# balazs-bamer/cdpr-simulation

Measured on AMD Instinct MI355X. Metric: CDPR sim-steps/sec (whole node), 65 536 parallel 8-cable robots, 1 ms dt, higher is better.
Workload: dtype f32

## Files before the change

### cdpr-simulation_amd/csrc/cdpr_onestep_kernel.hpp

```cpp
#pragma once
#include "cdpr_step_kernel.hpp"

namespace cdpr {

CDPR_DEV void row_to_lds(const float4* src, float4* dst_row) {
  __builtin_amdgcn_global_load_lds((const __attribute__((address_space(1))) void*)src, (__attribute__((address_space(3))) void*)dst_row, 16, 0, 0);
}


template <int NP, bool PR = false, bool FULL = false>
CDPR_DEV void pid_pairs(const StepArgs& a, int calls, bool is_vel, const v2f (&desired)[NP], const v2f (&actual)[NP], const v2f (&win)[NP][kWin],
                        v2f (&ierr)[NP], v2f (&f)[NP], v2f (&e_new)[NP], float& dbg_p, float& dbg_i, float& dbg_d, bool is_force = false) {
  const PidCoef c = pid_coef<PR>(a, is_vel);
  const bool run = (!PR || calls != 0) && !is_force;
  const bool full = FULL || calls >= c.nbuf;
  const float (&wt)[kWin + 2] = a.wrow;
  v2f error[NP], acc[NP];
#pragma unroll
  for (int k = 0; k < NP; ++k) {
    error[k] = desired[k] - actual[k];
    acc[k] = splat(wt[kWin]) * error[k];
  }
#pragma unroll
  for (int j = 0; j < kWin; ++j) {
#pragma unroll
    for (int k = 0; k < NP; ++k) acc[k] = fma2(wt[j], win[k][j], acc[k]);
  }
#pragma unroll
  for (int k = 0; k < NP; ++k) {
    const v2f p_term = splat(c.kp) * error[k];
    const v2f prev_ierr = ierr[k];
    v2f ie = fma2(a.dt, error[k], prev_ierr);
    const v2f i_term = splat(c.ki) * ie;
    const v2f i_cl = max2(min2(i_term, splat(c.imax)), splat(c.imin));
    const v2f ie_cl = i_cl * splat(c.inv_ki);
    ie.x = (i_cl.x != i_term.x) ? ie_cl.x : ie.x;
    ie.y = (i_cl.y != i_term.y) ? ie_cl.y : ie.y;
    const v2f derived = full ? acc[k] * splat(a.inv_dt) : splat(0.f);
    const v2f d_term = splat(c.kd) * derived;
    const v2f cmd = fma2(c.kf, desired[k], p_term) + i_cl + d_term;
    v2f out = c.clamp ? max2(min2(cmd, splat(c.cmax)), splat(c.cmin)) : cmd;
    const v2f bumped = fma2(splat(a.dt) * error[k], splat(c.ki), out);
    ie.x = (out.x != cmd.x) ? prev_ierr.x : ie.x;
    ie.y = (out.y != cmd.y) ? prev_ierr.y : ie.y;
    out.x = (out.x != cmd.x) ? bumped.x : out.x;
    out.y = (out.y != cmd.y) ? bumped.y : out.y;
    ierr[k] = run ? ie : prev_ierr;
    f[k] = run ? out : (is_force ? desired[k] : splat(0.f));
    e_new[k] = error[k];
    if (k == 0) {
      dbg_p = p_term.x;
      dbg_i = i_term.x;
      dbg_d = d_term.x;
    }
  }
}

typedef float f32x4 __attribute__((ext_vector_type(4)));
CDPR_DEV f32x4 load_slot_untracked(const float4* base, size_t stride, int slot, uint32_t off) {
  const char* p = reinterpret_cast<const char*>(base + (size_t)slot * stride) + off;
  f32x4 v;
  asm volatile("global_load_dwordx4 %0, %1, off" : "=a"(v) : "v"(p) : "memory");
  return v;
}
constexpr int vmcnt_imm(int n) { return (n & 15) | ((n >> 4) << 14) | (7 << 4) | (15 << 8); }

template <int N, bool FK, bool TD, bool PERSIST = false>
__global__ __launch_bounds__(64, 1) void cdpr_onestep_kernel(const StepArgs a_in) {
  const StepArgs& a = a_in;
  constexpr int NP = cable_pairs(N);
  constexpr int P = plat_slots(FK);
  constexpr int G = joint_groups(N);
  constexpr int NH = (NP + 1) / 2;
  constexpr int kCtrl = 5 * NP + NH;
  constexpr bool kCmdLds = (N % 4) == 0;
  constexpr int kCmdRows = kCmdLds ? N / 4 : 0;
  __shared__ __attribute__((aligned(16))) float lds[NP * kGeomFloatsPerPair];
  __shared__ float4 stage[kCtrl + (kCmdRows ? kCmdRows : 1)][64];

  const uint32_t lane = threadIdx.x;
  const size_t st0 = a.stride;
  const uint32_t nblocks = (a.batch + 63u) / 64u;
  uint32_t blk = blockIdx.x;
  uint32_t r = blk * 64u + lane;
  uint32_t rr = (r < a.batch) ? r : (a.batch - 1u);
  bool live = r < a.batch;
  uint32_t off = rr * 16u, woff = r * 16u;

  CDPR_STAMP(0);
  const float gval = (lane < NP * kGeomFloatsPerPair) ? a.geom[lane] : 0.f;
  float4 p0 = load_slot(a.state, st0, 0, off), p1 = load_slot(a.state, st0, 1, off), p2 = load_slot(a.state, st0, 2, off),
         p3 = load_slot(a.state, st0, 3, off);
  float4 p4 = make_float4(0.f, 0.f, 0.f, 1.f);
  if (FK) p4 = load_slot(a.state, st0, 4, off);
  if (lane < NP * kGeomFloatsPerPair) lds[lane] = gval;
  const bool force_mode = (a.flags & kFlagForceMode) != 0u;
  const bool first_world = (a.flags & kFlagFirstWorldStep) != 0u;
  const bool run_pid = !first_world && !force_mode && a.pid_calls != 0;
  bool staged = false;

  for (;;) {
  size_t st = st0;
  uint32_t goff = 0;
  if (PERSIST) asm volatile("" : "+s"(st), "+v"(goff));
  const float* const geo = lds + goff;
  const StepArgs a = block_args<PERSIST>(a_in);
  v2f desired[NP];
#pragma unroll
  for (int k = 0; k < NP; ++k) desired[k] = splat(0.f);
  const float* cp = a.cmd + (size_t)rr * N;
  if (!kCmdLds || force_mode) {
#pragma unroll
    for (int i = 0; i < N; ++i) {
      if (i & 1)
        desired[i / 2].y = cp[i];
      else
        desired[i / 2].x = cp[i];
    }
  }
  __builtin_amdgcn_fence(__ATOMIC_RELEASE, "wavefront");
  __builtin_amdgcn_wave_barrier();
  __builtin_amdgcn_fence(__ATOMIC_ACQUIRE, "wavefront");

  Platform s;
  unpack_platform(p0, p1, p2, p3.x, s);
  float fkx = p3.y, fky = p3.z, fkz = p3.w, fkqx = p4.x, fkqy = p4.y, fkqz = p4.z, fkqw = p4.w;

  {
    float keep = (s.px + s.qy) + (s.vy + s.wz) + fkqw;
#pragma unroll
    for (int k = 0; k < NP; ++k) keep += desired[k].x + desired[k].y;
    asm volatile("" ::"v"(keep));
    if (run_pid && !staged) {
#pragma unroll
      for (int j = 0; j < kCtrl; ++j)
        row_to_lds(reinterpret_cast<const float4*>(reinterpret_cast<const char*>(a.state + (size_t)(P + j) * st) + off), &stage[j][0]);
      if (kCmdLds) {
#pragma unroll
        for (int g = 0; g < kCmdRows; ++g) row_to_lds(reinterpret_cast<const float4*>(cp) + g, &stage[kCtrl + g][0]);
      }
    }
  }

  const uint32_t nblk = blk + gridDim.x;
  const bool more = PERSIST && nblk < nblocks;
  uint32_t nr = 0, nrr = 0;
  f32x4 n0 = {0.f, 0.f, 0.f, 0.f}, n1 = n0, n2 = n0, n3 = n0, n4 = {0.f, 0.f, 0.f, 1.f};
  if (PERSIST && more) {
    nr = nblk * 64u + lane;
    nrr = (nr < a.batch) ? nr : (a.batch - 1u);
    const uint32_t noff = nrr * 16u;
    n0 = load_slot_untracked(a.state, st, 0, noff), n1 = load_slot_untracked(a.state, st, 1, noff);
    n2 = load_slot_untracked(a.state, st, 2, noff), n3 = load_slot_untracked(a.state, st, 3, noff);
    if (FK) n4 = load_slot_untracked(a.state, st, 4, noff);
  }

  CDPR_STAMP(1);
  v2f len[NP], q[NP], qd[NP], jac[NP][6];
  {
    v2f l0[NP];
    ik_pairs<N, true>(geo, s.px, s.py, s.pz, s.qx, s.qy, s.qz, s.qw, len, jac, l0);
#pragma unroll
    for (int k = 0; k < NP; ++k) {
      q[k] = l0[k] - len[k];
      qd[k] = -fma2(s.wz, jac[k][5], fma2(s.wy, jac[k][4], fma2(s.wx, jac[k][3],
                    fma2(s.vz, jac[k][2], fma2(s.vy, jac[k][1], splat(s.vx) * jac[k][0])))));
    }
  }
  const bool publish = (a.publish_mask & 1ull) != 0ull;
  if (publish && live) {
    store_slot(a.obs, st, 0, woff, make_float4(s.px, s.py, s.pz, s.qx));
    store_slot(a.obs, st, 1, woff, make_float4(s.qy, s.qz, s.qw, s.vx));
    store_slot(a.obs, st, 2, woff, make_float4(s.vy, s.vz, s.wx, s.wy));
#pragma unroll
    for (int g = 0; g < G; ++g) {
      const int k0 = 2 * g, k1 = (2 * g + 1 < NP) ? 2 * g + 1 : 2 * g;
      const bool has = (2 * g + 1 < NP);
      store_slot(a.obs, st, 4 + g, woff, make_float4(q[k0].x, q[k0].y, has ? q[k1].x : 0.f, has ? q[k1].y : 0.f));
      store_slot(a.obs, st, 4 + G + g, woff, make_float4(qd[k0].x, qd[k0].y, has ? qd[k1].x : 0.f, has ? qd[k1].y : 0.f));
    }
  }

  CDPR_STAMP(2);
  float fk_res = 0.f;
  int fk_it = 0;
  v2f jest[NP][6];
  if (FK) {
    v2f elen[NP], unused[NP];
    bool active = true;
    for (int it = 0; it < a.fk_iters; ++it) {
      ik_pairs<N, false>(geo, fkx, fky, fkz, fkqx, fkqy, fkqz, fkqw, elen, jest, unused);
      v2f res[NP];
      v2f rm = splat(0.f);
#pragma unroll
      for (int k = 0; k < NP; ++k) {
        res[k] = len[k] - elen[k];
        rm = max2(rm, abs2(res[k]));
      }
      active = active && !(fmaxf(rm.x, rm.y) < a.fk_tol);
      float g[6];
      jt_times<NP>(jest, res, g);
      normal_solve<NP>(jest, a.fk_lambda, g);
      if (active) {
        fkx += g[0];
        fky += g[1];
        fkz += g[2];
        quat_apply_rotvec(fkqx, fkqy, fkqz, fkqw, g[3], g[4], g[5]);
        ++fk_it;
      }
    }
    ik_pairs<N, false>(geo, fkx, fky, fkz, fkqx, fkqy, fkqz, fkqw, elen, jest, unused);
    v2f rm = splat(0.f);
#pragma unroll
    for (int k = 0; k < NP; ++k) rm = max2(rm, abs2(len[k] - elen[k]));
    fk_res = fmaxf(rm.x, rm.y);
  }

  CDPR_STAMP(3);
  v2f f[NP], e_new[NP], ierr[NP];
#pragma unroll
  for (int k = 0; k < NP; ++k) {
    f[k] = splat(0.f);
    e_new[k] = splat(0.f);
    ierr[k] = splat(0.f);
  }
  float dbg_p = 0.f, dbg_i = 0.f, dbg_d = 0.f;
  bool dbg_wrote = false;
  if (run_pid) {
    __builtin_amdgcn_s_waitcnt(0x0F70);
    __builtin_amdgcn_fence(__ATOMIC_ACQUIRE, "wavefront");
    CDPR_STAMP(4);
    if (kCmdLds) {
#pragma unroll
      for (int g = 0; g < kCmdRows; ++g) {
        const float4 v = stage[kCtrl + g][lane];
        desired[2 * g] = (v2f){v.x, v.y};
        desired[2 * g + 1] = (v2f){v.z, v.w};
      }
    }
    v2f win[NP][kWin];
#pragma unroll
    for (int k = 0; k < NP; ++k) {
#pragma unroll
      for (int m = 0; m < 5; ++m) {
        const float4 w = stage[5 * k + m][lane];
        win[k][2 * m] = (v2f){w.x, w.y};
        win[k][2 * m + 1] = (v2f){w.z, w.w};
      }
    }
#pragma unroll
    for (int g = 0; g < NH; ++g) {
      const float4 h = stage[5 * NP + g][lane];
      ierr[2 * g] = (v2f){h.x, h.y};
      if (2 * g + 1 < NP) ierr[2 * g + 1] = (v2f){h.z, h.w};
    }
    const bool actual_is_vel = (a.flags & kFlagActualIsVelocity) != 0u;
    v2f actual[NP];
#pragma unroll
    for (int k = 0; k < NP; ++k) actual[k] = actual_is_vel ? qd[k] : q[k];
    const int ring_slot = a.ring_slot;
    pid_pairs<NP>(a, a.pid_calls, actual_is_vel, desired, actual, win, ierr, f, e_new, dbg_p, dbg_i, dbg_d);
    dbg_wrote = true;
    if (live) {
#pragma unroll
      for (int m = 0; m < 5; ++m) {
        if (m == (ring_slot >> 1)) {
#pragma unroll
          for (int k = 0; k < NP; ++k) CDPR_STORE_STATE(a.state, st, P + 5 * k + m, woff, ring_row(win[k], m, e_new[k], ring_slot));
        }
      }
#pragma unroll
      for (int g = 0; g < NH; ++g) {
        const int k1 = (2 * g + 1 < NP) ? 2 * g + 1 : 2 * g;
        CDPR_STORE_STATE(a.state, st, P + 5 * NP + g, woff, make_float4(ierr[2 * g].x, ierr[2 * g].y, ierr[k1].x, ierr[k1].y));
      }
    }
  }

  if (force_mode && !first_world) {
#pragma unroll
    for (int k = 0; k < NP; ++k) f[k] = desired[k];
  }

  if (PERSIST && more) {
    const uint32_t noff = nrr * 16u;
    if (run_pid) {
#pragma unroll
      for (int j = 0; j < kCtrl; ++j)
        row_to_lds(reinterpret_cast<const float4*>(reinterpret_cast<const char*>(a.state + (size_t)(P + j) * st) + noff), &stage[j][0]);
      if (kCmdLds) {
        const float* ncp = a.cmd + (size_t)nrr * N;
#pragma unroll
        for (int g = 0; g < kCmdRows; ++g) row_to_lds(reinterpret_cast<const float4*>(ncp) + g, &stage[kCtrl + g][0]);
      }
    }
  }

  CDPR_STAMP(5);
  v2f applied[NP];
  int td_flag = 0;
  if (TD) {
    v2f df[NP];
#pragma unroll
    for (int k = 0; k < NP; ++k) df[k] = f[k] - splat(a.td_mid);
    float g[6];
    if (FK) {
      jt_times<NP>(jest, df, g);
      normal_solve<NP, false>(jest, 0.f, g);
    } else {
      jt_times<NP>(jac, df, g);
      normal_solve<NP, false>(jac, 0.f, g);
    }
#pragma unroll
    for (int k = 0; k < NP; ++k) {
      v2f t = splat(a.td_mid);
#pragma unroll
      for (int c = 0; c < 6; ++c) t = fma2(g[c], FK ? jest[k][c] : jac[k][c], t);
      const v2f tc = max2(min2(t, splat(a.td_max)), splat(a.td_min));
      td_flag |= (tc.x != t.x) ? 1 : 0;
      if (2 * k + 1 < N) td_flag |= (tc.y != t.y) ? 1 : 0;
      applied[k] = tc;
    }
  } else {
#pragma unroll
    for (int k = 0; k < NP; ++k) applied[k] = f[k];
  }
  setforce_limits<NP>(a, qd, applied);

  if (a.dbg && live) write_pid_topic(a.dbg + (size_t)r * 9, dbg_wrote, dbg_wrote, dbg_p, dbg_i, dbg_d, desired[0].x, applied[0].x);
  if (publish && live) {
    store_slot(a.obs, st, 3, woff, make_float4(s.wz, fk_res, (float)fk_it, pack_flags(td_flag, travel_mask<N>(a, q))));
#pragma unroll
    for (int g = 0; g < G; ++g) {
      const int k0 = 2 * g, k1 = (2 * g + 1 < NP) ? 2 * g + 1 : 2 * g;
      const bool has = (2 * g + 1 < NP);
      store_slot(a.obs, st, 4 + 2 * G + g, woff,
                make_float4(applied[k0].x, applied[k0].y, has ? applied[k1].x : 0.f, has ? applied[k1].y : 0.f));
    }
  }

  CDPR_STAMP(6);
  {
    v2f tens[NP];
#pragma unroll
    for (int k = 0; k < NP; ++k) {
      tens[k] = fma2(-a.damping, qd[k], applied[k]);
      if (a.unilateral) tens[k] = max2(tens[k], splat(0.f));
    }
    if (FK) {
      uint32_t again = 0;
      asm volatile("" : "+v"(again));
      v2f len2[NP], l02[NP];
      ik_pairs<N, false>(lds + again, s.px, s.py, s.pz, s.qx, s.qy, s.qz, s.qw, len2, jac, l02);
    }
    float w[6];
    jt_times<NP>(jac, tens, w);
    w[0] = a.fgx - w[0];
    w[1] = a.fgy - w[1];
    w[2] = a.fgz - w[2];
    w[3] = -w[3];
    w[4] = -w[4];
    w[5] = -w[5];
    integrate(a, s, w);
  }
  if (PERSIST && more) {
    constexpr int kDmaOps = kCtrl + kCmdRows;
    static_assert(kDmaOps < 64, "vmcnt is a 6-bit counter");
    if (run_pid)
      __builtin_amdgcn_s_waitcnt(vmcnt_imm(kDmaOps));
    else
      __builtin_amdgcn_s_waitcnt(vmcnt_imm(0));
    asm volatile("" : "+a"(n0), "+a"(n1), "+a"(n2), "+a"(n3), "+a"(n4));
  }
  if (live) {
    CDPR_STORE_STATE(a.state, st, 0, woff, make_float4(s.px, s.py, s.pz, s.qx));
    CDPR_STORE_STATE(a.state, st, 1, woff, make_float4(s.qy, s.qz, s.qw, s.vx));
    CDPR_STORE_STATE(a.state, st, 2, woff, make_float4(s.vy, s.vz, s.wx, s.wy));
    CDPR_STORE_STATE(a.state, st, 3, woff, make_float4(s.wz, fkx, fky, fkz));
    if (FK) CDPR_STORE_STATE(a.state, st, 4, woff, make_float4(fkqx, fkqy, fkqz, fkqw));
  }
  CDPR_STAMP(7);
  if (!(PERSIST && more)) break;
  blk = nblk;
  r = nr;
  rr = nrr;
  live = r < a.batch;
  off = rr * 16u, woff = r * 16u;
  p0 = make_float4(n0.x, n0.y, n0.z, n0.w), p1 = make_float4(n1.x, n1.y, n1.z, n1.w), p2 = make_float4(n2.x, n2.y, n2.z, n2.w);
  p3 = make_float4(n3.x, n3.y, n3.z, n3.w), p4 = make_float4(n4.x, n4.y, n4.z, n4.w);
  staged = run_pid;
  }
}

#ifndef CDPR_CTL_LOAD_DELAY
#define CDPR_CTL_LOAD_DELAY 8
#endif
#ifndef CDPR_SPLIT_PRIO
#define CDPR_SPLIT_PRIO 1
#endif
#ifndef CDPR_STEADY_SHARED_IK
#define CDPR_STEADY_SHARED_IK 1
#endif
#ifndef CDPR_STEADY_NEWTON_WRITTEN_OUT
#define CDPR_STEADY_NEWTON_WRITTEN_OUT 1
#endif
constexpr int kIkRows = 7;
#ifdef CDPR_STAMPS
#define CDPR_SPLIT_STAMP(i)                                                                                          \
  do {                                                                                                               \
    __builtin_amdgcn_sched_barrier(0);                                                                               \
    if (a.stamps && lane == 0) a.stamps[(size_t)blockIdx.x * 8 + (i)] = __builtin_amdgcn_s_memrealtime();           \
    __builtin_amdgcn_sched_barrier(0);                                                                               \
  } while (0)
#else
#define CDPR_SPLIT_STAMP(i) do { } while (0)
#endif
#if defined(CDPR_STAMPS) && defined(CDPR_STAMPS_ITER)
#define CDPR_CTL_STAMP(i) do { } while (0)
#else
#define CDPR_CTL_STAMP(i) CDPR_SPLIT_STAMP(i)
#endif

template <int N, int XS, int ES, bool RAISED = true, bool STEADY = false>
CDPR_DEV void split_estimator_wave(const StepArgs& a, float* geo, float gval, uint32_t lane, bool live, size_t st, uint32_t off, uint32_t woff,
                                   const float4& p0, const float4& p1, const float4& p3, const v2f* x_force, v2f* x_tension, float* x_est,
                                   v2f* x_ik = nullptr) {
  constexpr int NP = cable_pairs(N);
#if defined(CDPR_STAMPS) && defined(CDPR_STAMPS_CLOCK)
  const unsigned long long clk0 = __builtin_amdgcn_s_memtime();
#endif
#if CDPR_SPLIT_PRIO == 1 || CDPR_SPLIT_PRIO == 4
  if (RAISED) __builtin_amdgcn_s_setprio(3);
#elif CDPR_SPLIT_PRIO == 3 || CDPR_SPLIT_PRIO == 5
  if (RAISED) __builtin_amdgcn_s_setprio(2);
#endif
  const float4 p4 = load_slot(a.state, st, 4, off);
  if (lane < NP * kGeomFloatsPerPair) geo[lane] = gval;
  __builtin_amdgcn_fence(__ATOMIC_RELEASE, "wavefront");
  __builtin_amdgcn_wave_barrier();
  __builtin_amdgcn_fence(__ATOMIC_ACQUIRE, "wavefront");
  float fkx = p3.y, fky = p3.z, fkz = p3.w, fkqx = p4.x, fkqy = p4.y, fkqz = p4.z, fkqw = p4.w;
  v2f len[NP];
  {
    v2f jac[NP][6], l0[NP];
    ik_pairs<N, false>(geo, p0.x, p0.y, p0.z, p0.w, p1.x, p1.y, p1.z, len, jac, l0);
    if (STEADY && CDPR_STEADY_SHARED_IK) {
#pragma unroll
      for (int k = 0; k < NP; ++k) {
        x_ik[(kIkRows * k) * 64 + lane] = len[k];
#pragma unroll
        for (int c = 0; c < 6; ++c) x_ik[(kIkRows * k + 1 + c) * 64 + lane] = jac[k][c];
      }
      __builtin_amdgcn_fence(__ATOMIC_RELEASE, "workgroup");
      __builtin_amdgcn_s_waitcnt(0xC07F);
      __builtin_amdgcn_s_barrier();
    }
  }
  float fk_res = 0.f;
  int fk_it = 0;
  v2f jest[NP][6];
  {
    v2f elen[NP], unused[NP];
    if (STEADY && CDPR_STEADY_NEWTON_WRITTEN_OUT) {
#pragma unroll
      for (int it = 0; it < 4; ++it) {
        ik_pairs<N, false>(geo, fkx, fky, fkz, fkqx, fkqy, fkqz, fkqw, elen, jest, unused);
        v2f res[NP];
#pragma unroll
        for (int k = 0; k < NP; ++k) res[k] = len[k] - elen[k];
        float g[6];
        jt_times<NP>(jest, res, g);
        normal_solve<NP>(jest, a.fk_lambda, g);
        fkx += g[0];
        fky += g[1];
        fkz += g[2];
        quat_apply_rotvec(fkqx, fkqy, fkqz, fkqw, g[3], g[4], g[5]);
#ifdef CDPR_STAMPS_ITER
        if (it < 3) {
          asm volatile("" ::"v"(fkqw));
          __builtin_amdgcn_sched_barrier(0);
          if (a.stamps && lane == 0) a.stamps[(size_t)blockIdx.x * 8 + 4 + it] = __builtin_amdgcn_s_memrealtime();
          __builtin_amdgcn_sched_barrier(0);
        }
#endif
      }
      fk_it = 4;
    } else {
      bool active = true;
      for (int it = 0; it < a.fk_iters; ++it) {
        ik_pairs<N, false>(geo, fkx, fky, fkz, fkqx, fkqy, fkqz, fkqw, elen, jest, unused);
        v2f res[NP];
        v2f rm = splat(0.f);
#pragma unroll
        for (int k = 0; k < NP; ++k) {
          res[k] = len[k] - elen[k];
          rm = max2(rm, abs2(res[k]));
        }
        active = active && !(fmaxf(rm.x, rm.y) < a.fk_tol);
        float g[6];
        jt_times<NP>(jest, res, g);
        normal_solve<NP>(jest, a.fk_lambda, g);
        if (active) {
          fkx += g[0];
          fky += g[1];
          fkz += g[2];
          quat_apply_rotvec(fkqx, fkqy, fkqz, fkqw, g[3], g[4], g[5]);
          ++fk_it;
        }
#ifdef CDPR_STAMPS_ITER
        if (it < 3) {
          asm volatile("" ::"v"(fkqw));
          __builtin_amdgcn_sched_barrier(0);
          if (a.stamps && lane == 0) a.stamps[(size_t)blockIdx.x * 8 + 4 + it] = __builtin_amdgcn_s_memrealtime();
          __builtin_amdgcn_sched_barrier(0);
        }
#endif
      }
    }
    ik_pairs<N, false>(geo, fkx, fky, fkz, fkqx, fkqy, fkqz, fkqw, elen, jest, unused);
    v2f rm = splat(0.f);
#pragma unroll
    for (int k = 0; k < NP; ++k) rm = max2(rm, abs2(len[k] - elen[k]));
    fk_res = fmaxf(rm.x, rm.y);
  }
  if (live) store_slot_aux<CDPR_SPLIT_PLAT_AUX>(a.state, st, 4, woff, make_float4(fkqx, fkqy, fkqz, fkqw));
  CDPR_SPLIT_STAMP(1);
  v2f td_l[6][3];
  float td_invd[6];
  normal_matrix_pk<NP, false>(jest, 0.f, td_l);
  chol_factor_pk(td_l, td_invd);
  __builtin_amdgcn_s_waitcnt(0xC07F);
  __builtin_amdgcn_s_barrier();
  CDPR_SPLIT_STAMP(2);
  __builtin_amdgcn_fence(__ATOMIC_ACQUIRE, "workgroup");
  v2f f[NP], df[NP], t_out[NP];
#pragma unroll
  for (int k = 0; k < NP; ++k) {
    f[k] = x_force[k * XS + lane];
    df[k] = f[k] - splat(a.td_mid);
  }
  int td_flag = 0;
  {
    float g[6];
    jt_times<NP>(jest, df, g);
    chol_apply_pk(td_l, td_invd, g);
#pragma unroll
    for (int k = 0; k < NP; ++k) {
      v2f t = splat(a.td_mid);
#pragma unroll
      for (int c = 0; c < 6; ++c) t = fma2(g[c], jest[k][c], t);
      const v2f tc = max2(min2(t, splat(a.td_max)), splat(a.td_min));
      td_flag |= (tc.x != t.x) ? 1 : 0;
      if (2 * k + 1 < N) td_flag |= (tc.y != t.y) ? 1 : 0;
      t_out[k] = tc;
    }
  }
#pragma unroll
  for (int k = 0; k < NP; ++k) x_tension[k * XS + lane] = t_out[k];
  x_est[0 * ES + lane] = fkx;
  x_est[1 * ES + lane] = fky;
  x_est[2 * ES + lane] = fkz;
  x_est[3 * ES + lane] = fk_res;
  x_est[4 * ES + lane] = (float)fk_it;
  x_est[5 * ES + lane] = (float)td_flag;
  __builtin_amdgcn_fence(__ATOMIC_RELEASE, "workgroup");
  __builtin_amdgcn_s_waitcnt(0xC07F);
  CDPR_SPLIT_STAMP(3);
#if defined(CDPR_STAMPS) && defined(CDPR_STAMPS_CLOCK)
  if (a.stamps && lane == 0) a.stamps[(size_t)blockIdx.x * 8 + 7] = __builtin_amdgcn_s_memtime() - clk0;
#endif
  __builtin_amdgcn_s_barrier();
}

template <int N, bool PR, bool STEADY, bool VEL>
CDPR_DEV void split_controller_wave(const StepArgs& a, float* geo, float gval, uint32_t lane, uint32_t r, uint32_t rr, bool live, size_t st, uint32_t off,
                                    uint32_t woff, const float4& p0, const float4& p1, const float4& p2, const float4& p3, v2f* x_force, const v2f* x_tension,
                                    const float* x_est, const v2f* x_ik = nullptr) {
  static_assert(!(STEADY && PR), "the steady instantiation serves uniform handles");
  constexpr int NP = cable_pairs(N);
  constexpr int P = plat_slots(true);
  constexpr int G = joint_groups(N);
  constexpr int NH = (NP + 1) / 2;
#if CDPR_SPLIT_PRIO == 2 || CDPR_SPLIT_PRIO == 5
  __builtin_amdgcn_s_setprio(3);
#endif
#if CDPR_CTL_LOAD_DELAY > 0
  __builtin_amdgcn_s_sleep(CDPR_CTL_LOAD_DELAY);
#endif
  float4 wraw[NP][5], hraw[NH];
#pragma unroll
  for (int k = 0; k < NP; ++k) {
#pragma unroll
    for (int m = 0; m < 5; ++m) wraw[k][m] = load_slot(a.state, st, P + 5 * k + m, off);
  }
#pragma unroll
  for (int g = 0; g < NH; ++g) hraw[g] = load_slot(a.state, st, P + 5 * NP + g, off);
  v2f desired[NP];
#pragma unroll
  for (int k = 0; k < NP; ++k) desired[k] = splat(0.f);
  const float* cp = a.cmd + (size_t)rr * N;
  if (N % 4 == 0) {
#pragma unroll
    for (int g = 0; g < N / 4; ++g) {
      const float4 v = reinterpret_cast<const float4*>(cp)[g];
      desired[2 * g] = (v2f){v.x, v.y};
      desired[2 * g + 1] = (v2f){v.z, v.w};
    }
  } else {
#pragma unroll
    for (int i = 0; i < N; ++i) {
      if (i & 1)
        desired[i / 2].y = cp[i];
      else
        desired[i / 2].x = cp[i];
    }
  }
  if (lane < NP * kGeomFloatsPerPair) geo[lane] = gval;
  __builtin_amdgcn_fence(__ATOMIC_RELEASE, "wavefront");
  __builtin_amdgcn_wave_barrier();
  __builtin_amdgcn_fence(__ATOMIC_ACQUIRE, "wavefront");

  Platform s;
  unpack_platform(p0, p1, p2, p3.x, s);

  v2f len[NP], q[NP], qd[NP], jac[NP][6];
  {
    v2f l0[NP];
    if (STEADY && CDPR_STEADY_SHARED_IK) {
      __builtin_amdgcn_s_barrier();
      __builtin_amdgcn_fence(__ATOMIC_ACQUIRE, "workgroup");
#pragma unroll
      for (int k = 0; k < NP; ++k) {
        len[k] = x_ik[(kIkRows * k) * 64 + lane];
#pragma unroll
        for (int c = 0; c < 6; ++c) jac[k][c] = x_ik[(kIkRows * k + 1 + c) * 64 + lane];
        l0[k] = *reinterpret_cast<const v2f*>(geo + k * kGeomFloatsPerPair + 12);
      }
    } else {
      ik_pairs<N, true>(geo, s.px, s.py, s.pz, s.qx, s.qy, s.qz, s.qw, len, jac, l0);
    }
#pragma unroll
    for (int k = 0; k < NP; ++k) {
      q[k] = l0[k] - len[k];
      qd[k] = -fma2(s.wz, jac[k][5], fma2(s.wy, jac[k][4], fma2(s.wx, jac[k][3],
                    fma2(s.vz, jac[k][2], fma2(s.vy, jac[k][1], splat(s.vx) * jac[k][0])))));
    }
  }
  const bool publish = STEADY || (a.publish_mask & 1ull) != 0ull;
  if (publish && live) {
    store_slot(a.obs, st, 0, woff, make_float4(s.px, s.py, s.pz, s.qx));
    store_slot(a.obs, st, 1, woff, make_float4(s.qy, s.qz, s.qw, s.vx));
    store_slot(a.obs, st, 2, woff, make_float4(s.vy, s.vz, s.wx, s.wy));
#pragma unroll
    for (int g = 0; g < G; ++g) {
      const int k0 = 2 * g, k1 = (2 * g + 1 < NP) ? 2 * g + 1 : 2 * g;
      const bool has = (2 * g + 1 < NP);
      store_slot(a.obs, st, 4 + g, woff, make_float4(q[k0].x, q[k0].y, has ? q[k1].x : 0.f, has ? q[k1].y : 0.f));
      store_slot(a.obs, st, 4 + G + g, woff, make_float4(qd[k0].x, qd[k0].y, has ? qd[k1].x : 0.f, has ? qd[k1].y : 0.f));
    }
  }

  v2f f[NP], e_new[NP], ierr[NP];
#pragma unroll
  for (int k = 0; k < NP; ++k) {
    f[k] = splat(0.f);
    e_new[k] = splat(0.f);
    ierr[k] = (k & 1) ? (v2f){hraw[k / 2].z, hraw[k / 2].w} : (v2f){hraw[k / 2].x, hraw[k / 2].y};
  }
  float dbg_p = 0.f, dbg_i = 0.f, dbg_d = 0.f;
  bool dbg_wrote = false;
  const bool first_world = !STEADY && (a.flags & kFlagFirstWorldStep) != 0u;
  uint32_t meta = 0u;
  if (PR) meta = a.meta[rr];
  const int calls = PR ? (int)(meta >> kMetaCallShift) : a.pid_calls;
  if (PR && live && !first_world) a.meta[r] = (uint8_t)((meta & kMetaModeMask) | ((uint32_t)min(calls + 1, (int)kMetaCallMax) << kMetaCallShift));
  const bool force_mode = !STEADY && !PR && (a.flags & kFlagForceMode) != 0u;
  if (force_mode && !first_world) {
#pragma unroll
    for (int k = 0; k < NP; ++k) f[k] = desired[k];
  } else if (STEADY || (!first_world && (PR || calls != 0))) {
    v2f win[NP][kWin];
#pragma unroll
    for (int k = 0; k < NP; ++k) {
#pragma unroll
      for (int m = 0; m < 5; ++m) {
        win[k][2 * m] = (v2f){wraw[k][m].x, wraw[k][m].y};
        win[k][2 * m + 1] = (v2f){wraw[k][m].z, wraw[k][m].w};
      }
    }
    const bool actual_is_vel = STEADY ? VEL : PR ? ((meta & kMetaModeMask) == kMetaVelocity) : ((a.flags & kFlagActualIsVelocity) != 0u);
    v2f actual[NP];
#pragma unroll
    for (int k = 0; k < NP; ++k) actual[k] = actual_is_vel ? qd[k] : q[k];
    const int ring_slot = a.ring_slot;
    const bool is_force = PR && (meta & kMetaModeMask) == kMetaForce;
#if CDPR_SPLIT_PRIO == 3 || CDPR_SPLIT_PRIO == 4
    __builtin_amdgcn_s_setprio(3);
#endif
    pid_pairs<NP, PR, STEADY>(a, calls, actual_is_vel, desired, actual, win, ierr, f, e_new, dbg_p, dbg_i, dbg_d, is_force);
    dbg_wrote = (!PR || calls != 0) && !is_force;
    if (live) {
#pragma unroll
      for (int m = 0; m < 5; ++m) {
        if (m == (ring_slot >> 1)) {
          if (!STEADY) {
#pragma unroll
            for (int k = 0; k < NP; ++k) CDPR_STORE_STATE(a.state, st, P + 5 * k + m, woff, ring_row(win[k], m, e_new[k], ring_slot));
          } else if (ring_slot & 1) {
#pragma unroll
            for (int k = 0; k < NP; ++k) CDPR_STORE_STATE(a.state, st, P + 5 * k + m, woff, make_float4(win[k][2 * m].x, win[k][2 * m].y, e_new[k].x, e_new[k].y));
          } else {
#pragma unroll
            for (int k = 0; k < NP; ++k) CDPR_STORE_STATE(a.state, st, P + 5 * k + m, woff, make_float4(e_new[k].x, e_new[k].y, win[k][2 * m + 1].x, win[k][2 * m + 1].y));
          }
        }
      }
#pragma unroll
      for (int g = 0; g < NH; ++g) {
        const int k1 = (2 * g + 1 < NP) ? 2 * g + 1 : 2 * g;
        CDPR_STORE_STATE(a.state, st, P + 5 * NP + g, woff, make_float4(ierr[2 * g].x, ierr[2 * g].y, ierr[k1].x, ierr[k1].y));
      }
    }
  }
#pragma unroll
  for (int k = 0; k < NP; ++k) x_force[k * 64 + lane] = f[k];
  __builtin_amdgcn_fence(__ATOMIC_RELEASE, "workgroup");
  __builtin_amdgcn_s_waitcnt(0xC07F);
  CDPR_CTL_STAMP(4);
#if CDPR_SPLIT_PRIO >= 3
  __builtin_amdgcn_s_setprio(0);
#endif
  __builtin_amdgcn_s_barrier();
  __builtin_amdgcn_s_barrier();
  CDPR_CTL_STAMP(5);
  __builtin_amdgcn_fence(__ATOMIC_ACQUIRE, "workgroup");
  v2f applied[NP];
#pragma unroll
  for (int k = 0; k < NP; ++k) applied[k] = x_tension[k * 64 + lane];
  const float fkx = x_est[0 * 64 + lane], fky = x_est[1 * 64 + lane], fkz = x_est[2 * 64 + lane], fk_res = x_est[3 * 64 + lane],
              fk_it = x_est[4 * 64 + lane], td_flag = x_est[5 * 64 + lane];
  setforce_limits<NP>(a, qd, applied);
  if (!STEADY && a.dbg && live) write_pid_topic(a.dbg + (size_t)r * 9, dbg_wrote, dbg_wrote, dbg_p, dbg_i, dbg_d, desired[0].x, applied[0].x);
  if (publish && live) {
    store_slot(a.obs, st, 3, woff, make_float4(s.wz, fk_res, fk_it, (!STEADY && a.travel_on) ? pack_flags((int)td_flag, travel_mask<N>(a, q)) : td_flag));
#pragma unroll
    for (int g = 0; g < G; ++g) {
      const int k0 = 2 * g, k1 = (2 * g + 1 < NP) ? 2 * g + 1 : 2 * g;
      const bool has = (2 * g + 1 < NP);
      store_slot(a.obs, st, 4 + 2 * G + g, woff,
                 make_float4(applied[k0].x, applied[k0].y, has ? applied[k1].x : 0.f, has ? applied[k1].y : 0.f));
    }
  }
  {
    v2f tens[NP];
#pragma unroll
    for (int k = 0; k < NP; ++k) {
      tens[k] = fma2(-a.damping, qd[k], applied[k]);
      if (a.unilateral) tens[k] = max2(tens[k], splat(0.f));
    }
    float w[6];
    jt_times<NP>(jac, tens, w);
    w[0] = a.fgx - w[0];
    w[1] = a.fgy - w[1];
    w[2] = a.fgz - w[2];
    w[3] = -w[3];
    w[4] = -w[4];
    w[5] = -w[5];
    integrate(a, s, w);
  }
  if (live) {
    store_slot_aux<CDPR_SPLIT_PLAT_AUX>(a.state, st, 0, woff, make_float4(s.px, s.py, s.pz, s.qx));
    store_slot_aux<CDPR_SPLIT_PLAT_AUX>(a.state, st, 1, woff, make_float4(s.qy, s.qz, s.qw, s.vx));
    store_slot_aux<CDPR_SPLIT_PLAT_AUX>(a.state, st, 2, woff, make_float4(s.vy, s.vz, s.wx, s.wy));
    store_slot_aux<CDPR_SPLIT_PLAT_AUX>(a.state, st, 3, woff, make_float4(s.wz, fkx, fky, fkz));
  }
  CDPR_CTL_STAMP(6);
}

template <int N, bool PR, bool STEADY, bool VEL>
CDPR_DEV void split_kernel_body(const StepArgs& a) {
  constexpr int NP = cable_pairs(N);
  __shared__ __attribute__((aligned(16))) float lds[2][NP * kGeomFloatsPerPair];
  __shared__ v2f x_force[NP][64];
  __shared__ v2f x_tension[NP][64];
  __shared__ float x_est[6][64];
  v2f* x_ik = nullptr;
  if constexpr (STEADY && CDPR_STEADY_SHARED_IK) {
    __shared__ v2f ik_rows_at_state[kIkRows * NP][64];
    x_ik = &ik_rows_at_state[0][0];
  }

  const uint32_t swap = __builtin_popcount(blockIdx.x & a.split_swap) & 1u;
  const uint32_t wave = (threadIdx.x >> 6) ^ swap, lane = threadIdx.x & 63u;
  const uint32_t r = blockIdx.x * 64u + lane;
  const uint32_t rr = (r < a.batch) ? r : (a.batch - 1u);
  const bool live = r < a.batch;
  const size_t st = a.stride;
  const uint32_t off = rr * 16u, woff = r * 16u;
  float* const geo = lds[wave];

  if (wave == 0) CDPR_SPLIT_STAMP(0);
#ifdef CDPR_STAMPS
  if (a.stamps && lane == 0)
    reinterpret_cast<uint32_t*>(&a.stamps[(size_t)blockIdx.x * 8 + 7])[threadIdx.x >> 6] =
        (__builtin_amdgcn_s_getreg((16 - 1) << 11 | 4) & 0xffffu) | ((__builtin_amdgcn_s_getreg((4 - 1) << 11 | 20) & 0xfu) << 16);
#endif
  const float gval = (lane < NP * kGeomFloatsPerPair) ? a.geom[lane] : 0.f;
  const float4 p0 = load_slot(a.state, st, 0, off), p1 = load_slot(a.state, st, 1, off), p2 = load_slot(a.state, st, 2, off),
               p3 = load_slot(a.state, st, 3, off);
  if (wave == 0) {
    split_estimator_wave<N, 64, 64, true, STEADY>(a, geo, gval, lane, live, st, off, woff, p0, p1, p3, &x_force[0][0], &x_tension[0][0], &x_est[0][0], x_ik);
    return;
  }
  split_controller_wave<N, PR, STEADY, VEL>(a, geo, gval, lane, r, rr, live, st, off, woff, p0, p1, p2, p3, &x_force[0][0], &x_tension[0][0], &x_est[0][0], x_ik);
}
template <int N, bool PR = false>
__global__ __launch_bounds__(128, 2) void cdpr_split_kernel(const StepArgs a) { split_kernel_body<N, PR, false, false>(a); }
template <int N, bool VEL>
__global__ __launch_bounds__(128, 2) void cdpr_split_steady_kernel(const StepArgs a) { split_kernel_body<N, false, true, VEL>(a); }

}
```

Measured before the change: 6.832 billion.

## Specialize steady split kernel: shared rotation, vectorized IK rows, half-row ring stores

In the steady instantiation, the estimator wave builds the rotation matrix once, runs a specialized IK that reads geometry as float4 from LDS, and publishes the nine rotation entries to LDS. The controller wave reuses them in a new integrator instead of recomputing the rotation. The ring-buffer history write becomes a single 64-bit buffer store of the new error pair in place of full float4 row rewrites. Clamps are done with inline asm min/max, and asm register pins constrain instruction scheduling. The changes add LDS footprint and code complexity, and the pins and asm may keep the compiler from reordering or fusing instructions.

```diff
diff --git a/cdpr-simulation_amd/csrc/cdpr_onestep_kernel.hpp b/cdpr-simulation_amd/csrc/cdpr_onestep_kernel.hpp
--- a/cdpr-simulation_amd/csrc/cdpr_onestep_kernel.hpp
+++ b/cdpr-simulation_amd/csrc/cdpr_onestep_kernel.hpp
@@ -7,6 +7,100 @@
   __builtin_amdgcn_global_load_lds((const __attribute__((address_space(1))) void*)src, (__attribute__((address_space(3))) void*)dst_row, 16, 0, 0);
 }
 
+
+#ifndef CDPR_STEADY_PIN
+#define CDPR_STEADY_PIN 1
+#endif
+CDPR_LEAF float cdpr_pin(float v) {
+#if CDPR_STEADY_PIN
+  asm("" : "+v"(v));
+#endif
+  return v;
+}
+
+template <int NP, bool ODD>
+CDPR_DEV void steady_ik_rows(const float* lds, const Rot& r, float px, float py, float pz, v2f (&len)[NP], v2f (&jac)[NP][6]) {
+#pragma unroll
+  for (int k = 0; k < NP; ++k) {
+    const float4 g0 = *reinterpret_cast<const float4*>(lds + k * kGeomFloatsPerPair);
+    const float4 g1 = *reinterpret_cast<const float4*>(lds + k * kGeomFloatsPerPair + 4);
+    const float4 g2 = *reinterpret_cast<const float4*>(lds + k * kGeomFloatsPerPair + 8);
+    const v2f ax = {g0.x, g0.y}, ay = {g0.z, g0.w}, az = {g1.x, g1.y};
+    const v2f bx = {g1.z, g1.w}, by = {g2.x, g2.y}, bz = {g2.z, g2.w};
+    const v2f rbx = fma2(r.r02, bz, fma2(r.r01, by, splat(r.r00) * bx));
+    const v2f rby = fma2(r.r12, bz, fma2(r.r11, by, splat(r.r10) * bx));
+    const v2f rbz = fma2(r.r22, bz, fma2(r.r21, by, splat(r.r20) * bx));
+    const v2f lx = (rbx - ax) + splat(px), ly = (rby - ay) + splat(py), lz = (rbz - az) + splat(pz);
+    const v2f l2 = fma2(lz, lz, fma2(ly, ly, lx * lx));
+    const v2f inv = rsq2(l2);
+    len[k] = l2 * inv;
+    const v2f ux = lx * inv, uy = ly * inv, uz = lz * inv;
+    jac[k][0] = ux;
+    jac[k][1] = uy;
+    jac[k][2] = uz;
+    jac[k][3] = fma2(rby, uz, -(rbz * uy));
+    jac[k][4] = fma2(rbz, ux, -(rbx * uz));
+    jac[k][5] = fma2(rbx, uy, -(rby * ux));
+    if (ODD && k == NP - 1) {
+      const float4 g3 = *reinterpret_cast<const float4*>(lds + k * kGeomFloatsPerPair + 12);
+      const v2f mask = {g3.z, g3.w};
+      len[k] *= mask;
+#pragma unroll
+      for (int c = 0; c < 6; ++c) jac[k][c] *= mask;
+    }
+  }
+}
+CDPR_DEV void steady_world_step(const StepArgs& a, Platform& s, const float (&w)[6], const Rot& r) {
+  const auto P = [](float v) { return cdpr_pin(v); };
+  s.vx = fmaf(a.dt_inv_mass, w[0], s.vx);
+  s.vy = fmaf(a.dt_inv_mass, w[1], s.vy);
+  s.vz = fmaf(a.dt_inv_mass, w[2], s.vz);
+  float tbx = P(fmaf(r.r20, w[5], P(fmaf(r.r10, w[4], P(r.r00 * w[3])))));
+  float tby = P(fmaf(r.r21, w[5], P(fmaf(r.r11, w[4], P(r.r01 * w[3])))));
+  float tbz = P(fmaf(r.r22, w[5], P(fmaf(r.r12, w[4], P(r.r02 * w[3])))));
+  const float obx = P(fmaf(r.r20, s.wz, P(fmaf(r.r10, s.wy, P(r.r00 * s.wx)))));
+  const float oby = P(fmaf(r.r21, s.wz, P(fmaf(r.r11, s.wy, P(r.r01 * s.wx)))));
+  const float obz = P(fmaf(r.r22, s.wz, P(fmaf(r.r12, s.wy, P(r.r02 * s.wx)))));
+  const float iox = P(fmaf(a.ib[4], obz, P(fmaf(a.ib[3], oby, P(a.ib[0] * obx)))));
+  const float ioy = P(fmaf(a.ib[5], obz, P(fmaf(a.ib[1], oby, P(a.ib[3] * obx)))));
+  const float ioz = P(fmaf(a.ib[2], obz, P(fmaf(a.ib[5], oby, P(a.ib[4] * obx)))));
+  tbx = P(tbx - P(fmaf(oby, ioz, -P(obz * ioy))));
+  tby = P(tby - P(fmaf(obz, iox, -P(obx * ioz))));
+  tbz = P(tbz - P(fmaf(obx, ioy, -P(oby * iox))));
+  const float abx = P(fmaf(a.ibinv[4], tbz, P(fmaf(a.ibinv[3], tby, P(a.ibinv[0] * tbx)))));
+  const float aby = P(fmaf(a.ibinv[5], tbz, P(fmaf(a.ibinv[1], tby, P(a.ibinv[3] * tbx)))));
+  const float abz = P(fmaf(a.ibinv[2], tbz, P(fmaf(a.ibinv[5], tby, P(a.ibinv[4] * tbx)))));
+  s.wx = P(fmaf(a.dt, P(fmaf(r.r02, abz, P(fmaf(r.r01, aby, P(r.r00 * abx))))), s.wx));
+  s.wy = P(fmaf(a.dt, P(fmaf(r.r12, abz, P(fmaf(r.r11, aby, P(r.r10 * abx))))), s.wy));
+  s.wz = P(fmaf(a.dt, P(fmaf(r.r22, abz, P(fmaf(r.r21, aby, P(r.r20 * abx))))), s.wz));
+  s.px = P(fmaf(a.dt, s.vx, s.px));
+  s.py = P(fmaf(a.dt, s.vy, s.py));
+  s.pz = P(fmaf(a.dt, s.vz, s.pz));
+  const float h = a.half_dt;
+  const float nx = P(fmaf(h, P(fmaf(-s.wz, s.qy, P(fmaf(s.wy, s.qz, P(s.qw * s.wx))))), s.qx));
+  const float ny = P(fmaf(h, P(fmaf(-s.wx, s.qz, P(fmaf(s.wz, s.qx, P(s.qw * s.wy))))), s.qy));
+  const float nz = P(fmaf(h, P(fmaf(-s.wy, s.qx, P(fmaf(s.wx, s.qy, P(s.qw * s.wz))))), s.qz));
+  const float nw = P(fmaf(-h, P(fmaf(s.wz, s.qz, P(fmaf(s.wy, s.qy, P(s.wx * s.qx))))), s.qw));
+  const float inv = P(__frsqrt_rn(fmaf(nw, nw, fmaf(nz, nz, fmaf(ny, ny, nx * nx)))));
+  s.qx = P(nx * inv);
+  s.qy = P(ny * inv);
+  s.qz = P(nz * inv);
+  s.qw = P(nw * inv);
+}
+CDPR_DEV void store_ring_half(float4* base, size_t stride, int slot, uint32_t off, uint32_t half, v2f v) {
+  typedef unsigned int u32x2 __attribute__((ext_vector_type(2)));
+  const u32x2 d = __builtin_bit_cast(u32x2, v);
+  const auto rsrc = __builtin_amdgcn_make_buffer_rsrc(base + (size_t)slot * stride, 0, (int)(stride * sizeof(float4)), 0x00020000);
+  __builtin_amdgcn_raw_buffer_store_b64(d, rsrc, off, half, CDPR_STORE_AUX);
+}
+CDPR_LEAF v2f steady_clamp2(v2f v, float hi, float lo) {
+  v2f r;
+  asm("v_min_f32_e32 %0, %1, %2" : "=v"(r.x) : "v"(v.x), "v"(hi));
+  asm("v_min_f32_e32 %0, %1, %2" : "=v"(r.y) : "v"(v.y), "v"(hi));
+  asm("v_max_f32_e32 %0, %1, %2" : "=v"(r.x) : "v"(r.x), "v"(lo));
+  asm("v_max_f32_e32 %0, %1, %2" : "=v"(r.y) : "v"(r.y), "v"(lo));
+  return r;
+}
 
 template <int NP, bool PR = false, bool FULL = false>
 CDPR_DEV void pid_pairs(const StepArgs& a, int calls, bool is_vel, const v2f (&desired)[NP], const v2f (&actual)[NP], const v2f (&win)[NP][kWin],
@@ -15,6 +109,7 @@
   const bool run = (!PR || calls != 0) && !is_force;
   const bool full = FULL || calls >= c.nbuf;
   const float (&wt)[kWin + 2] = a.wrow;
+  const float cmax_q = FULL ? __builtin_canonicalizef(c.cmax) : c.cmax, cmin_q = FULL ? __builtin_canonicalizef(c.cmin) : c.cmin;
   v2f error[NP], acc[NP];
 #pragma unroll
   for (int k = 0; k < NP; ++k) {
@@ -39,7 +134,7 @@
     const v2f derived = full ? acc[k] * splat(a.inv_dt) : splat(0.f);
     const v2f d_term = splat(c.kd) * derived;
     const v2f cmd = fma2(c.kf, desired[k], p_term) + i_cl + d_term;
-    v2f out = c.clamp ? max2(min2(cmd, splat(c.cmax)), splat(c.cmin)) : cmd;
+    v2f out = c.clamp ? (FULL ? steady_clamp2(cmd, cmax_q, cmin_q) : max2(min2(cmd, splat(c.cmax)), splat(c.cmin))) : cmd;
     const v2f bumped = fma2(splat(a.dt) * error[k], splat(c.ki), out);
     ie.x = (out.x != cmd.x) ? prev_ierr.x : ie.x;
     ie.y = (out.y != cmd.y) ? prev_ierr.y : ie.y;
@@ -404,7 +499,47 @@
 #ifndef CDPR_STEADY_NEWTON_WRITTEN_OUT
 #define CDPR_STEADY_NEWTON_WRITTEN_OUT 1
 #endif
+#ifndef CDPR_STEADY_RING_HALF
+#define CDPR_STEADY_RING_HALF 1
+#endif
 constexpr int kIkRows = 7;
+
+CDPR_DEV Rot steady_quat_to_rot(float x, float y, float z, float w) {
+  const float x2 = cdpr_pin(x + x), y2 = cdpr_pin(y + y), z2 = cdpr_pin(z + z);
+  const float xx = cdpr_pin(x * x2), yy = cdpr_pin(y * y2), zz = cdpr_pin(z * z2);
+  const float xy = cdpr_pin(x * y2), xz = cdpr_pin(x * z2), yz = cdpr_pin(y * z2);
+  const float wx = cdpr_pin(w * x2), wy = cdpr_pin(w * y2), wz = cdpr_pin(w * z2);
+  Rot r;
+  r.r00 = cdpr_pin(1.f - cdpr_pin(yy + zz));
+  r.r01 = cdpr_pin(xy - wz);
+  r.r02 = cdpr_pin(xz + wy);
+  r.r10 = cdpr_pin(xy + wz);
+  r.r11 = cdpr_pin(1.f - cdpr_pin(xx + zz));
+  r.r12 = cdpr_pin(yz - wx);
+  r.r20 = cdpr_pin(xz - wy);
+  r.r21 = cdpr_pin(yz + wx);
+  r.r22 = cdpr_pin(1.f - cdpr_pin(xx + yy));
+  return r;
+}
+CDPR_DEV void steady_quat_apply_rotvec(float& qx, float& qy, float& qz, float& qw, float tx, float ty, float tz) {
+  const float a2 = fmaf(tz, tz, fmaf(ty, ty, tx * tx));
+  const float inv_a = __frsqrt_rn(fmaxf(a2, 1e-30f));
+  float s, c;
+  __sincosf(0.5f * (a2 * inv_a), &s, &c);
+  const bool tiny = a2 < 1e-8f;
+  const float k = cdpr_pin(tiny ? fmaf(a2, -1.f / 48.f, 0.5f) : s * inv_a);
+  const float cw = cdpr_pin(tiny ? fmaf(a2, -0.125f, 1.f) : c);
+  const float dx = cdpr_pin(k * tx), dy = cdpr_pin(k * ty), dz = cdpr_pin(k * tz);
+  const float nw = cdpr_pin(fmaf(-dz, qz, cdpr_pin(fmaf(-dy, qy, cdpr_pin(fmaf(-dx, qx, cdpr_pin(cw * qw)))))));
+  const float nx = cdpr_pin(fmaf(-dz, qy, cdpr_pin(fmaf(dy, qz, cdpr_pin(fmaf(qw, dx, cdpr_pin(cw * qx)))))));
+  const float ny = cdpr_pin(fmaf(-dx, qz, cdpr_pin(fmaf(dz, qx, cdpr_pin(fmaf(qw, dy, cdpr_pin(cw * qy)))))));
+  const float nz = cdpr_pin(fmaf(-dy, qx, cdpr_pin(fmaf(dx, qy, cdpr_pin(fmaf(qw, dz, cdpr_pin(cw * qz)))))));
+  const float inv = cdpr_pin(__frsqrt_rn(fmaf(nw, nw, fmaf(nz, nz, fmaf(ny, ny, nx * nx)))));
+  qx = cdpr_pin(nx * inv);
+  qy = cdpr_pin(ny * inv);
+  qz = cdpr_pin(nz * inv);
+  qw = cdpr_pin(nw * inv);
+}
 #ifdef CDPR_STAMPS
 #define CDPR_SPLIT_STAMP(i)                                                                                          \
   do {                                                                                                               \
@@ -424,8 +559,9 @@
 template <int N, int XS, int ES, bool RAISED = true, bool STEADY = false>
 CDPR_DEV void split_estimator_wave(const StepArgs& a, float* geo, float gval, uint32_t lane, bool live, size_t st, uint32_t off, uint32_t woff,
                                    const float4& p0, const float4& p1, const float4& p3, const v2f* x_force, v2f* x_tension, float* x_est,
-                                   v2f* x_ik = nullptr) {
+                                   v2f* x_ik = nullptr, float* x_rot = nullptr) {
   constexpr int NP = cable_pairs(N);
+  constexpr bool ODD = (N & 1) != 0;
 #if defined(CDPR_STAMPS) && defined(CDPR_STAMPS_CLOCK)
   const unsigned long long clk0 = __builtin_amdgcn_s_memtime();
 #endif
@@ -443,8 +579,18 @@
   v2f len[NP];
   {
     v2f jac[NP][6], l0[NP];
-    ik_pairs<N, false>(geo, p0.x, p0.y, p0.z, p0.w, p1.x, p1.y, p1.z, len, jac, l0);
     if (STEADY && CDPR_STEADY_SHARED_IK) {
+      const Rot r0 = steady_quat_to_rot(p0.w, p1.x, p1.y, p1.z);
+      steady_ik_rows<NP, ODD>(geo, r0, p0.x, p0.y, p0.z, len, jac);
+      x_rot[0 * 64 + lane] = r0.r00;
+      x_rot[1 * 64 + lane] = r0.r01;
+      x_rot[2 * 64 + lane] = r0.r02;
+      x_rot[3 * 64 + lane] = r0.r10;
+      x_rot[4 * 64 + lane] = r0.r11;
+      x_rot[5 * 64 + lane] = r0.r12;
+      x_rot[6 * 64 + lane] = r0.r20;
+      x_rot[7 * 64 + lane] = r0.r21;
+      x_rot[8 * 64 + lane] = r0.r22;
 #pragma unroll
       for (int k = 0; k < NP; ++k) {
         x_ik[(kIkRows * k) * 64 + lane] = len[k];
@@ -454,6 +600,8 @@
       __builtin_amdgcn_fence(__ATOMIC_RELEASE, "workgroup");
       __builtin_amdgcn_s_waitcnt(0xC07F);
       __builtin_amdgcn_s_barrier();
+    } else {
+      ik_pairs<N, false>(geo, p0.x, p0.y, p0.z, p0.w, p1.x, p1.y, p1.z, len, jac, l0);
     }
   }
   float fk_res = 0.f;
@@ -464,7 +612,7 @@
     if (STEADY && CDPR_STEADY_NEWTON_WRITTEN_OUT) {
 #pragma unroll
       for (int it = 0; it < 4; ++it) {
-        ik_pairs<N, false>(geo, fkx, fky, fkz, fkqx, fkqy, fkqz, fkqw, elen, jest, unused);
+        steady_ik_rows<NP, ODD>(geo, steady_quat_to_rot(fkqx, fkqy, fkqz, fkqw), fkx, fky, fkz, elen, jest);
         v2f res[NP];
 #pragma unroll
         for (int k = 0; k < NP; ++k) res[k] = len[k] - elen[k];
@@ -474,7 +622,7 @@
         fkx += g[0];
         fky += g[1];
         fkz += g[2];
-        quat_apply_rotvec(fkqx, fkqy, fkqz, fkqw, g[3], g[4], g[5]);
+        steady_quat_apply_rotvec(fkqx, fkqy, fkqz, fkqw, g[3], g[4], g[5]);
 #ifdef CDPR_STAMPS_ITER
         if (it < 3) {
           asm volatile("" ::"v"(fkqw));
@@ -517,7 +665,10 @@
 #endif
       }
     }
-    ik_pairs<N, false>(geo, fkx, fky, fkz, fkqx, fkqy, fkqz, fkqw, elen, jest, unused);
+    if (STEADY && CDPR_STEADY_NEWTON_WRITTEN_OUT)
+      steady_ik_rows<NP, ODD>(geo, steady_quat_to_rot(fkqx, fkqy, fkqz, fkqw), fkx, fky, fkz, elen, jest);
+    else
+      ik_pairs<N, false>(geo, fkx, fky, fkz, fkqx, fkqy, fkqz, fkqw, elen, jest, unused);
     v2f rm = splat(0.f);
 #pragma unroll
     for (int k = 0; k < NP; ++k) rm = max2(rm, abs2(len[k] - elen[k]));
@@ -575,7 +726,7 @@
 template <int N, bool PR, bool STEADY, bool VEL>
 CDPR_DEV void split_controller_wave(const StepArgs& a, float* geo, float gval, uint32_t lane, uint32_t r, uint32_t rr, bool live, size_t st, uint32_t off,
                                     uint32_t woff, const float4& p0, const float4& p1, const float4& p2, const float4& p3, v2f* x_force, const v2f* x_tension,
-                                    const float* x_est, const v2f* x_ik = nullptr) {
+                                    const float* x_est, const v2f* x_ik = nullptr, const float* x_rot = nullptr) {
   static_assert(!(STEADY && PR), "the steady instantiation serves uniform handles");
   constexpr int NP = cable_pairs(N);
   constexpr int P = plat_slots(true);
@@ -706,14 +857,20 @@
           if (!STEADY) {
 #pragma unroll
             for (int k = 0; k < NP; ++k) CDPR_STORE_STATE(a.state, st, P + 5 * k + m, woff, ring_row(win[k], m, e_new[k], ring_slot));
-          } else if (ring_slot & 1) {
-#pragma unroll
-            for (int k = 0; k < NP; ++k) CDPR_STORE_STATE(a.state, st, P + 5 * k + m, woff, make_float4(win[k][2 * m].x, win[k][2 * m].y, e_new[k].x, e_new[k].y));
-          } else {
-#pragma unroll
-            for (int k = 0; k < NP; ++k) CDPR_STORE_STATE(a.state, st, P + 5 * k + m, woff, make_float4(e_new[k].x, e_new[k].y, win[k][2 * m + 1].x, win[k][2 * m + 1].y));
+          } else if (!CDPR_STEADY_RING_HALF) {
+            if (ring_slot & 1) {
+#pragma unroll
+              for (int k = 0; k < NP; ++k) CDPR_STORE_STATE(a.state, st, P + 5 * k + m, woff, make_float4(win[k][2 * m].x, win[k][2 * m].y, e_new[k].x, e_new[k].y));
+            } else {
+#pragma unroll
+              for (int k = 0; k < NP; ++k) CDPR_STORE_STATE(a.state, st, P + 5 * k + m, woff, make_float4(e_new[k].x, e_new[k].y, win[k][2 * m + 1].x, win[k][2 * m + 1].y));
+            }
           }
         }
+      }
+      if (STEADY && CDPR_STEADY_RING_HALF) {
+#pragma unroll
+        for (int k = 0; k < NP; ++k) store_ring_half(a.state, st, P + 5 * k + (ring_slot >> 1), woff, (uint32_t)(ring_slot & 1) * 8u, e_new[k]);
       }
 #pragma unroll
       for (int g = 0; g < NH; ++g) {
@@ -739,7 +896,22 @@
   for (int k = 0; k < NP; ++k) applied[k] = x_tension[k * 64 + lane];
   const float fkx = x_est[0 * 64 + lane], fky = x_est[1 * 64 + lane], fkz = x_est[2 * 64 + lane], fk_res = x_est[3 * 64 + lane],
               fk_it = x_est[4 * 64 + lane], td_flag = x_est[5 * 64 + lane];
-  setforce_limits<NP>(a, qd, applied);
+  if (STEADY) {
+    if (a.vel_limit > 0.f) {
+#pragma unroll
+      for (int k = 0; k < NP; ++k) {
+        applied[k].x = (qd[k].x > a.vel_limit && applied[k].x > 0.f) || (qd[k].x < -a.vel_limit && applied[k].x < 0.f) ? 0.f : applied[k].x;
+        applied[k].y = (qd[k].y > a.vel_limit && applied[k].y > 0.f) || (qd[k].y < -a.vel_limit && applied[k].y < 0.f) ? 0.f : applied[k].y;
+      }
+    }
+    if (a.effort >= 0.f) {
+      const float hi = __builtin_canonicalizef(a.effort), lo = __builtin_canonicalizef(-a.effort);
+#pragma unroll
+      for (int k = 0; k < NP; ++k) applied[k] = steady_clamp2(applied[k], hi, lo);
+    }
+  } else {
+    setforce_limits<NP>(a, qd, applied);
+  }
   if (!STEADY && a.dbg && live) write_pid_topic(a.dbg + (size_t)r * 9, dbg_wrote, dbg_wrote, dbg_p, dbg_i, dbg_d, desired[0].x, applied[0].x);
   if (publish && live) {
     store_slot(a.obs, st, 3, woff, make_float4(s.wz, fk_res, fk_it, (!STEADY && a.travel_on) ? pack_flags((int)td_flag, travel_mask<N>(a, q)) : td_flag));
@@ -756,7 +928,12 @@
 #pragma unroll
     for (int k = 0; k < NP; ++k) {
       tens[k] = fma2(-a.damping, qd[k], applied[k]);
-      if (a.unilateral) tens[k] = max2(tens[k], splat(0.f));
+      if (!STEADY && a.unilateral) tens[k] = max2(tens[k], splat(0.f));
+    }
+    if (STEADY && a.unilateral) {
+      asm volatile("" ::: "memory");
+#pragma unroll
+      for (int k = 0; k < NP; ++k) tens[k] = max2(tens[k], splat(0.f));
     }
     float w[6];
     jt_times<NP>(jac, tens, w);
@@ -766,7 +943,21 @@
     w[3] = -w[3];
     w[4] = -w[4];
     w[5] = -w[5];
-    integrate(a, s, w);
+    if (STEADY && CDPR_STEADY_SHARED_IK) {
+      Rot r;
+      r.r00 = x_rot[0 * 64 + lane];
+      r.r01 = x_rot[1 * 64 + lane];
+      r.r02 = x_rot[2 * 64 + lane];
+      r.r10 = x_rot[3 * 64 + lane];
+      r.r11 = x_rot[4 * 64 + lane];
+      r.r12 = x_rot[5 * 64 + lane];
+      r.r20 = x_rot[6 * 64 + lane];
+      r.r21 = x_rot[7 * 64 + lane];
+      r.r22 = x_rot[8 * 64 + lane];
+      steady_world_step(a, s, w, r);
+    } else {
+      integrate(a, s, w);
+    }
   }
   if (live) {
     store_slot_aux<CDPR_SPLIT_PLAT_AUX>(a.state, st, 0, woff, make_float4(s.px, s.py, s.pz, s.qx));
@@ -785,9 +976,12 @@
   __shared__ v2f x_tension[NP][64];
   __shared__ float x_est[6][64];
   v2f* x_ik = nullptr;
+  float* x_rot = nullptr;
   if constexpr (STEADY && CDPR_STEADY_SHARED_IK) {
     __shared__ v2f ik_rows_at_state[kIkRows * NP][64];
+    __shared__ float rot_at_state[9][64];
     x_ik = &ik_rows_at_state[0][0];
+    x_rot = &rot_at_state[0][0];
   }
 
   const uint32_t swap = __builtin_popcount(blockIdx.x & a.split_swap) & 1u;
@@ -809,10 +1003,10 @@
   const float4 p0 = load_slot(a.state, st, 0, off), p1 = load_slot(a.state, st, 1, off), p2 = load_slot(a.state, st, 2, off),
                p3 = load_slot(a.state, st, 3, off);
   if (wave == 0) {
-    split_estimator_wave<N, 64, 64, true, STEADY>(a, geo, gval, lane, live, st, off, woff, p0, p1, p3, &x_force[0][0], &x_tension[0][0], &x_est[0][0], x_ik);
+    split_estimator_wave<N, 64, 64, true, STEADY>(a, geo, gval, lane, live, st, off, woff, p0, p1, p3, &x_force[0][0], &x_tension[0][0], &x_est[0][0], x_ik, x_rot);
     return;
   }
-  split_controller_wave<N, PR, STEADY, VEL>(a, geo, gval, lane, r, rr, live, st, off, woff, p0, p1, p2, p3, &x_force[0][0], &x_tension[0][0], &x_est[0][0], x_ik);
+  split_controller_wave<N, PR, STEADY, VEL>(a, geo, gval, lane, r, rr, live, st, off, woff, p0, p1, p2, p3, &x_force[0][0], &x_tension[0][0], &x_est[0][0], x_ik, x_rot);
 }
 template <int N, bool PR = false>
 __global__ __launch_bounds__(128, 2) void cdpr_split_kernel(const StepArgs a) { split_kernel_body<N, PR, false, false>(a); }
```

Result: no change. 6.828 billion, median of 2 (-0.1%).
